# QWERTY6191/projected-lmc

Measured on AMD Instinct MI355X. Metric: MLL+grad iters/sec, n=8192 16-task LMC, higher is better.
Workload: dtype f32; 1 GPU; C3: ProjectedGPModel+ProjectedLMCmll exact training step (PLMC_fast), n=8192 d=8 p=16 q=8 Matern-5/2 fp32; latents sharded q/N per GPU; n_points=8192, n_dim=8, n_tasks=16, n_latents=8, parallelism=latent-shard x1

## Files before the change

projected-lmc_amd/csrc/api.hip:

```cpp
#include <stdlib.h>
#include <mutex>
#include <vector>

#include "api_common.hpp"
#include "../../include/plmc.h"

namespace plmc {
char *err_buf() {
  static thread_local char buf[256] = {0};
  return buf;
}

static const char *kProfNames[PK_COUNT] = {"k_assemble", "k_write_rhs", "k_assemble_cross", "k_diag",   "k_panel",
                                           "k_trail",    "k_wdiag",     "k_trtri_row",      "k_extract_col",
                                           "k_wt_matvec", "k_kinv_grad", "k_reduce_grad", "k_kernel_vjp",
                                           "sweep_total", "k_trail_row", "k_trail_head", "k_gpanel", "k_kacc", "k_grad_tiles", "k_split_w", "k_posterior_moments"};
struct ProfRec { int id; hipEvent_t a, b; double flops, bytes; };
static unsigned g_prof_mask = 0;
static std::vector<ProfRec> g_recs;
static std::vector<hipEvent_t> g_free;

static hipEvent_t get_event() {
  if (!g_free.empty()) { hipEvent_t e = g_free.back(); g_free.pop_back(); return e; }
  hipEvent_t e;
  if (hipEventCreate(&e) != hipSuccess) return nullptr;
  return e;
}

static std::recursive_mutex g_api_mutex;
void api_lock() { g_api_mutex.lock(); }
void api_unlock() { g_api_mutex.unlock(); }

static Knobs g_knobs;
static bool g_knobs_loaded = false;
static void load_knobs() {
  const char *h = getenv("PLMC_HALF_TILES"), *g = getenv("PLMC_GRP"), *o = getenv("PLMC_KINV_ORDER");
  g_knobs.half_tiles = h ? (atoi(h) == 1 ? 1e30 : (double)atoi(h)) : 640.0;
  g_knobs.grp = g ? atoi(g) : 0;
  g_knobs.serial = getenv("PLMC_SERIAL") && atoi(getenv("PLMC_SERIAL")) != 0;
  g_knobs.kinv_order = o ? atoi(o) : 4;
  g_knobs.bulk_lds = getenv("PLMC_BULK_LDS") ? atoi(getenv("PLMC_BULK_LDS")) : -1;
  g_knobs.split = getenv("PLMC_SPLIT") ? atoi(getenv("PLMC_SPLIT")) : 2;
  if (g_knobs.split != 0 && g_knobs.split != 3) g_knobs.split = 2;
  g_knobs.bulk_streams = getenv("PLMC_BULK_STREAMS") ? atoi(getenv("PLMC_BULK_STREAMS")) : 2;
  g_knobs.chain = getenv("PLMC_CHAIN") ? atoi(getenv("PLMC_CHAIN")) : 1;
  g_knobs.chain_nw = getenv("PLMC_CHAIN_NW") ? atoi(getenv("PLMC_CHAIN_NW")) : 0;
  g_knobs.chain_edge = getenv("PLMC_CHAIN_EDGE") ? atoi(getenv("PLMC_CHAIN_EDGE")) : 0;
  g_knobs_loaded = true;
}
const Knobs &knobs() {
  if (!g_knobs_loaded) {
    std::lock_guard<std::recursive_mutex> lk(g_api_mutex);
    if (!g_knobs_loaded) load_knobs();
  }
  return g_knobs;
}

constexpr int SWEEP_CTX = 2;
struct SweepCtx {
  hipStream_t caller = nullptr;
  bool used = false;
  unsigned long long stamp = 0;
  hipStream_t side[3] = {nullptr, nullptr, nullptr};
  hipEvent_t ev[16] = {nullptr};
};
static SweepCtx g_ctx[64][SWEEP_CTX];
static unsigned long long g_stamp = 0;
static thread_local int t_ctx = 0;
static SweepCtx *cur_ctx() {
  int dev = 0;
  if (hipGetDevice(&dev) != hipSuccess || dev < 0 || dev >= 64) return nullptr;
  return &g_ctx[dev][t_ctx];
}
hipStream_t side_stream(int which) {
  SweepCtx *c = cur_ctx();
  if (!c || which < 0 || which > 2) return nullptr;
  if (!c->side[which]) {
    int lo = 0, hi = 0;
    (void)hipDeviceGetStreamPriorityRange(&lo, &hi);
    if (hipStreamCreateWithPriority(&c->side[which], hipStreamNonBlocking, which == 2 ? lo : hi) != hipSuccess) c->side[which] = nullptr;
  }
  return c->side[which];
}
hipEvent_t sync_event(int idx) {
  SweepCtx *c = cur_ctx();
  if (!c) return nullptr;
  hipEvent_t &e = c->ev[idx & 15];
  if (!e && hipEventCreateWithFlags(&e, hipEventDisableTiming) != hipSuccess) e = nullptr;
  return e;
}
void bind_sweep_ctx(hipStream_t caller, int e_prev_idx) {
  int dev = 0;
  if (hipGetDevice(&dev) != hipSuccess || dev < 0 || dev >= 64) { t_ctx = 0; return; }
  SweepCtx *set = g_ctx[dev];
  int pick = -1;
  for (int i = 0; i < SWEEP_CTX; ++i)
    if (set[i].used && set[i].caller == caller) pick = i;
  if (pick < 0) {
    for (int i = 0; i < SWEEP_CTX && pick < 0; ++i)
      if (!set[i].used) pick = i;
    if (pick < 0) {
      pick = 0;
      for (int i = 1; i < SWEEP_CTX; ++i)
        if (set[i].stamp < set[pick].stamp) pick = i;
      if (set[pick].ev[e_prev_idx & 15]) (void)hipStreamWaitEvent(caller, set[pick].ev[e_prev_idx & 15], 0);
    }
    set[pick].caller = caller;
    set[pick].used = true;
  }
  set[pick].stamp = ++g_stamp;
  t_ctx = pick;
}

template <typename T>
__global__ __launch_bounds__(NTHREADS) void k_mfma_rate(T *sink, int iters) {
  using Tr = Traits<T>;
  typename Tr::acc_t acc[16];
#pragma unroll
  for (int i = 0; i < 16; ++i)
#pragma unroll
    for (int r = 0; r < 4; ++r) acc[i][r] = T(0);
  T a[4], b[4];
#pragma unroll
  for (int i = 0; i < 4; ++i) { a[i] = T(1) + T(threadIdx.x & 7) * T(1e-3) + T(i); b[i] = T(0.5) - T(i) * T(1e-3); }
#pragma unroll 1
  for (int it = 0; it < iters; ++it) {
#pragma unroll
    for (int i = 0; i < 16; ++i) acc[i] = Tr::mfma(a[i >> 2], b[i & 3], acc[i]);
  }
  T s = T(0);
#pragma unroll
  for (int i = 0; i < 16; ++i) s += acc[i][0] + acc[i][1] + acc[i][2] + acc[i][3];
  sink[(size_t)blockIdx.x * NTHREADS + threadIdx.x] = s;
}

typedef __bf16 rate_bf16x8 __attribute__((ext_vector_type(8)));
__global__ __launch_bounds__(NTHREADS) void k_mfma_rate_bf16(float *sink, int iters) {
  f32x4 acc[16];
#pragma unroll
  for (int i = 0; i < 16; ++i)
#pragma unroll
    for (int r = 0; r < 4; ++r) acc[i][r] = 0.f;
  rate_bf16x8 a[4], b[4];
#pragma unroll
  for (int i = 0; i < 4; ++i)
#pragma unroll
    for (int j = 0; j < 8; ++j) { a[i][j] = (__bf16)(1.0f + 0.01f * (float)((threadIdx.x + j) & 7) + (float)i); b[i][j] = (__bf16)(0.5f - 0.01f * (float)(i + j)); }
#pragma unroll 1
  for (int it = 0; it < iters; ++it) {
#pragma unroll
    for (int i = 0; i < 16; ++i) acc[i] = __builtin_amdgcn_mfma_f32_16x16x32_bf16(a[i >> 2], b[i & 3], acc[i], 0, 0, 0);
  }
  float s = 0.f;
#pragma unroll
  for (int i = 0; i < 16; ++i) s += acc[i][0] + acc[i][1] + acc[i][2] + acc[i][3];
  sink[(size_t)blockIdx.x * NTHREADS + threadIdx.x] = s;
}

template <typename T, bool BF16 = false> static int mfma_rate_impl(void *sink, int64_t sink_bytes, double *tflops) {
  int dev = 0;
  hipDeviceProp_t prop;
  if (hipGetDevice(&dev) != hipSuccess || hipGetDeviceProperties(&prop, dev) != hipSuccess) return fail("plmc_prof_mfma_rate", "no device");
  const int grid = 4 * prop.multiProcessorCount, iters = 4000;
  if (!sink || !tflops || sink_bytes < (int64_t)grid * NTHREADS * (int64_t)sizeof(T)) return fail("plmc_prof_mfma_rate", "sink too small");
  hipEvent_t e0 = nullptr, e1 = nullptr;
  if (hipEventCreate(&e0) != hipSuccess || hipEventCreate(&e1) != hipSuccess) return fail("plmc_prof_mfma_rate", "event");
  double best = 0.0;
  for (int rep = 0; rep < 3; ++rep) {
    (void)hipEventRecord(e0, nullptr);
    if (BF16) hipLaunchKernelGGL(k_mfma_rate_bf16, dim3(grid), dim3(NTHREADS), 0, nullptr, (float *)sink, iters);
    else hipLaunchKernelGGL(k_mfma_rate<T>, dim3(grid), dim3(NTHREADS), 0, nullptr, (T *)sink, iters);
    (void)hipEventRecord(e1, nullptr);
    float ms = 0.f;
    if (hipEventSynchronize(e1) != hipSuccess || hipEventElapsedTime(&ms, e0, e1) != hipSuccess) break;
    const double fl = (double)grid * (NTHREADS / 64) * (double)iters * 16.0 * 2.0 * 16 * 16 * (BF16 ? 32 : 4);
    if (ms > 0.f && fl / (ms * 1e-3) / 1e12 > best) best = fl / (ms * 1e-3) / 1e12;
  }
  (void)hipEventDestroy(e0);
  (void)hipEventDestroy(e1);
  *tflops = best;
  return launch_status("plmc_prof_mfma_rate");
}

ProfScope::ProfScope(int id, hipStream_t st, double flops, double bytes) : idx_(-1), st_(st) {
  api_lock();
  if (!((g_prof_mask >> id) & 1u) || g_recs.size() >= (1u << 20)) return;
  ProfRec r{id, get_event(), get_event(), flops, bytes};
  if (!r.a || !r.b) return;
  (void)hipEventRecord(r.a, st);
  g_recs.push_back(r);
  idx_ = (long)g_recs.size() - 1;
}
ProfScope::~ProfScope() {
// ... 46 lines not shown
```

projected-lmc_amd/csrc/api_common.hpp:

```cpp
#pragma once
#include <hip/hip_runtime.h>
#include <stdint.h>
#include <stdio.h>
#include <string.h>

#include "gemm_core.hpp"

namespace plmc {

constexpr int MAX_DIM = 32;

char *err_buf();

inline int fail(const char *fn, const char *msg) {
  snprintf(err_buf(), 256, "%s: %s", fn, msg);
  return -1;
}

inline int launch_status(const char *fn) {
  hipError_t e = hipGetLastError();
  if (e != hipSuccess) {
    snprintf(err_buf(), 256, "%s: HIP launch failed: %s", fn, hipGetErrorString(e));
    return -2;
  }
  return 0;
}

#define PLMC_REQUIRE(cond, msg) \
  do { if (!(cond)) return plmc::fail(__func__, msg); } while (0)

enum ProfKernel { PK_ASSEMBLE, PK_WRITE_RHS, PK_CROSS, PK_DIAG, PK_PANEL, PK_TRAIL, PK_WDIAG, PK_TRTRI, PK_EXTRACT,
                  PK_WTMV, PK_KINV_GRAD, PK_REDUCE, PK_VJP, PK_SWEEP, PK_TRAIL_ROW, PK_TRAIL_HEAD, PK_GPANEL, PK_KACC, PK_GRAD_TILES, PK_SPLIT, PK_POST, PK_COUNT };

struct ProfScope {
  ProfScope(int id, hipStream_t st, double flops, double bytes);
  ~ProfScope();
  long idx_;
  hipStream_t st_;
};

struct Knobs {
  double half_tiles;
  int grp;
  bool serial;
  int bulk_lds;
  int split;
  int bulk_streams;
  int chain;
  int chain_edge;
  int chain_nw;
  int kinv_order;
};
const Knobs &knobs();

struct AssembleJob {
  int kind, n, d;
  const void *X, *ell, *oscale, *noise;
};
int assemble_rows(const AssembleJob &job, int elem_bytes, void *A, int64_t lda, int64_t strideA, int q, int ib0, int nrows, void *stream,
                  int ncols = -1, int skip = 0);

hipStream_t side_stream(int which = 0);
hipEvent_t sync_event(int idx);
void bind_sweep_ctx(hipStream_t caller, int e_prev_idx);

inline bool aligned16(const void *p) { return (reinterpret_cast<uintptr_t>(p) & 15) == 0; }

}
```

projected-lmc_amd/csrc/bf3_engine.hpp:

```cpp
#pragma once
#include "gemm_core.hpp"

namespace plmc {

constexpr int B3_NT = 512;
constexpr int B3_K = 32;
constexpr int B3_AW = 256, B3_BW = 128;
constexpr int B3_A_PLANE = (B3_K / 8) * B3_AW * 16;
constexpr int B3_B_PLANE = (B3_K / 8) * B3_BW * 16;
constexpr int B3_WB_BYTES = 64 * 132 * 4;

typedef __bf16 b3_bf16x8 __attribute__((ext_vector_type(8)));
typedef _Float16 b3_f16x8 __attribute__((ext_vector_type(8)));
typedef short b3_s16x8 __attribute__((ext_vector_type(8)));

struct SplitB3 {
  static constexpr int NPL = 3;
  static constexpr float LEVEL1 = 1.0f;
  typedef b3_bf16x8 frag_t;
  static __device__ __forceinline__ f32x4 mfma(frag_t a, frag_t b, f32x4 c) { return __builtin_amdgcn_mfma_f32_16x16x32_bf16(a, b, c, 0, 0, 0); }
  static __device__ __forceinline__ void split(float v, short (&o)[3]) {
    const __bf16 a = (__bf16)v;
    const float r1 = v - (float)a;
    const __bf16 b = (__bf16)r1;
    const __bf16 c = (__bf16)(r1 - (float)b);
    o[0] = __builtin_bit_cast(short, a); o[1] = __builtin_bit_cast(short, b); o[2] = __builtin_bit_cast(short, c);
  }
};
struct SplitH2 {
  static constexpr int NPL = 2;
  static constexpr float LEVEL1 = 1.0f / 2048.0f;
  typedef b3_f16x8 frag_t;
  static __device__ __forceinline__ f32x4 mfma(frag_t a, frag_t b, f32x4 c) { return __builtin_amdgcn_mfma_f32_16x16x32_f16(a, b, c, 0, 0, 0); }
  static __device__ __forceinline__ void split(float v, short (&o)[2]) {
    const _Float16 a = (_Float16)v;
    const _Float16 b = (_Float16)((v - (float)a) * 2048.0f);
    o[0] = __builtin_bit_cast(short, a); o[1] = __builtin_bit_cast(short, b);
  }
};
template <class S> constexpr int b3_stage_bytes() { return S::NPL * (B3_A_PLANE + B3_B_PLANE); }
template <class S> constexpr int b3_lds_bytes() { return 2 * b3_stage_bytes<S>() > 2 * B3_WB_BYTES ? 2 * b3_stage_bytes<S>() : 2 * B3_WB_BYTES; }

template <class S> __host__ __device__ inline int64_t b3_index(int64_t k, int plane, int64_t col, int64_t ld) {
  return (((k >> 3) * S::NPL + plane) * ld + col) * 8 + (k & 7);
}
template <class S> __host__ __device__ inline int64_t b3_elems(int64_t rows, int64_t ld) { return rows * S::NPL * ld; }

__host__ __device__ inline float b3_scale_for(float bound) {
  int e;
  (void)frexpf(bound, &e);
  return ldexpf(1.0f, 13 - e);
}

template <class S>
__device__ __forceinline__ void b3_split_store(const float (&x)[8][4], unsigned short *dst, int64_t ld, float scale) {
#pragma unroll
  for (int c = 0; c < 4; ++c) {
    b3_s16x8 pl[S::NPL];
#pragma unroll
    for (int r = 0; r < 8; ++r) {
      short o[S::NPL];
      S::split(x[r][c] * scale, o);
#pragma unroll
      for (int p = 0; p < S::NPL; ++p) pl[p][r] = o[p];
    }
#pragma unroll
    for (int p = 0; p < S::NPL; ++p) *reinterpret_cast<b3_s16x8 *>(dst + (int64_t)p * ld * 8 + c * 8) = pl[p];
  }
}

template <class S, bool COPY>
__device__ __forceinline__ void b3_split_block(const float *__restrict__ Sp, int64_t lds_, unsigned short *__restrict__ P, int64_t ld, float scale,
                                               float *D, int64_t ldd, int tid) {
#pragma unroll 1
  for (int w = tid; w < 16 * 32; w += NTHREADS) {
    const int k8 = w >> 5, c4 = (w & 31) * 4;
    float x[8][4];
#pragma unroll
    for (int r = 0; r < 8; ++r) {
      const float4 v = *reinterpret_cast<const float4 *>(Sp + (int64_t)(k8 * 8 + r) * lds_ + c4);
      x[r][0] = v.x; x[r][1] = v.y; x[r][2] = v.z; x[r][3] = v.w;
      if (COPY) *reinterpret_cast<float4 *>(D + (int64_t)(k8 * 8 + r) * ldd + c4) = v;
    }
    b3_split_store<S>(x, P + ((int64_t)k8 * S::NPL * ld + c4) * 8, ld, scale);
  }
}

struct B3NoPre { __device__ __forceinline__ void operator()() const {} };
template <class S, int NSTG = 2, int NPRE = 0, class PRE = B3NoPre, bool REV = false>
__device__ __forceinline__ void b3_mainloop(Acc<float> &acc0, Acc<float> &acc1, const unsigned short *__restrict__ Ap, int64_t lda_,
                                            const unsigned short *__restrict__ Bp, int64_t ldb_, int K, unsigned char *lds, PRE pre = PRE()) {
  static_assert(NPRE == 0 || (NPRE == 8 && NSTG == 2), "pre-loads: eight, two-stage loop only");
  constexpr int NPL = S::NPL, STAGE = b3_stage_bytes<S>();
  typedef typename S::frag_t frag_t;
  const int tid = threadIdx.x, lane = tid & 63;
  const int w = __builtin_amdgcn_readfirstlane(tid >> 6);
  const int half = w >> 2, wm = (w >> 1) & 1, wn = w & 1;
  const unsigned RSA = (unsigned)(NPL * lda_ * 16), RSB = (unsigned)(NPL * ldb_ * 16);
  const unsigned PLA = (unsigned)(lda_ * 16), PLB = (unsigned)(ldb_ * 16);
  const unsigned gA0 = (unsigned)(w >> 2) * RSA + (unsigned)(w & 3) * 1024u;
  const unsigned gB0 = (unsigned)((w >> 1) & 3) * RSB + (unsigned)(w & 1) * 1024u;
  const unsigned lA0 = (unsigned)(((w >> 2) * B3_AW + (w & 3) * 64) * 16);
  const unsigned lB0 = (unsigned)(NPL * B3_A_PLANE + (((w >> 1) & 3) * B3_BW + (w & 1) * 64) * 16);
  const unsigned voff = (unsigned)lane * 16u;
  const int64_t fwdA = (int64_t)(B3_K / 8) * RSA, fwdB = (int64_t)(B3_K / 8) * RSB;
  const int64_t stepA = REV ? -fwdA : fwdA, stepB = REV ? -fwdB : fwdB;
  const char *baseA = reinterpret_cast<const char *>(Ap) + (REV ? (int64_t)(K / B3_K - 1) * fwdA : 0);
  const char *baseB = reinterpret_cast<const char *>(Bp) + (REV ? (int64_t)(K / B3_K - 1) * fwdB : 0);
  typedef __attribute__((address_space(3))) void lds_void;
  auto issue = [&](int buf) {
    const __amdgpu_buffer_rsrc_t rA = __builtin_amdgcn_make_buffer_rsrc(const_cast<char *>(baseA), 0, 0x7fffffff, 0x00020000);
    const __amdgpu_buffer_rsrc_t rB = __builtin_amdgcn_make_buffer_rsrc(const_cast<char *>(baseB), 0, 0x7fffffff, 0x00020000);
    unsigned char *sb = lds + buf * STAGE;
#pragma unroll
    for (int j = 0; j < 2 * NPL; ++j)
      __builtin_amdgcn_raw_ptr_buffer_load_lds(rA, (lds_void *)(sb + lA0 + (j >> 1) * B3_A_PLANE + (j & 1) * (2 * B3_AW * 16)), 16, voff,
                                               gA0 + (unsigned)(j & 1) * 2u * RSA + (unsigned)(j >> 1) * PLA, 0, 0);
#pragma unroll
    for (int j = 0; j < NPL; ++j)
      __builtin_amdgcn_raw_ptr_buffer_load_lds(rB, (lds_void *)(sb + lB0 + j * B3_B_PLANE), 16, voff, gB0 + (unsigned)j * PLB, 0, 0);
    baseA += stepA;
    baseB += stepB;
  };
  const int kg = lane >> 4, fr = lane & 15;
  const unsigned aA = (unsigned)((kg * B3_AW + half * 128 + wm * 64 + fr) * 16);
  const unsigned aB = (unsigned)(NPL * B3_A_PLANE + (kg * B3_BW + wn * 64 + fr) * 16);
  auto compute = [&](int buf) {
    const unsigned char *sa = lds + buf * STAGE + aA, *sb = lds + buf * STAGE + aB;
    auto fa = [&](int plane, frag_t (&f)[4]) {
#pragma unroll
      for (int t = 0; t < 4; ++t) f[t] = *reinterpret_cast<const frag_t *>(sa + plane * B3_A_PLANE + t * 256);
    };
    auto fb = [&](int plane, frag_t (&f)[4]) {
#pragma unroll
      for (int t = 0; t < 4; ++t) f[t] = *reinterpret_cast<const frag_t *>(sb + plane * B3_B_PLANE + t * 256);
    };
    auto mm = [&](Acc<float> &acc, const frag_t (&x)[4], const frag_t (&y)[4]) {
#pragma unroll
      for (int mt = 0; mt < 4; ++mt)
#pragma unroll
        for (int nt = 0; nt < 4; ++nt) acc.v[mt][nt] = S::mfma(x[mt], y[nt], acc.v[mt][nt]);
    };
    if constexpr (NPL == 3) {
      frag_t bh[4], bx[4], ax[4], ay[4];
      fb(0, bh);
      fa(2, ax);
      mm(acc1, ax, bh);
      fa(1, ay);
      mm(acc1, ay, bh);
      fb(1, bx);
      mm(acc1, ay, bx);
      fa(0, ax);
      mm(acc1, ax, bx);
      fb(2, bx);
      mm(acc1, ax, bx);
      mm(acc0, ax, bh);
    } else {
      frag_t b0[4], b1[4], a0[4], a1[4];
      fb(0, b0);
      fa(1, a1);
      mm(acc1, a1, b0);
      fa(0, a0);
      fb(1, b1);
      mm(acc1, a0, b1);
      mm(acc0, a0, b0);
    }
  };
  const int nst = K / B3_K;
  if constexpr (NSTG == 2) {
    issue(0);
#pragma unroll 1
    for (int s = 0; s + 2 < nst; s += 2) {
      __syncthreads();
      issue(1);
      compute(0);
      __syncthreads();
      issue(0);
      compute(1);
    }
    __syncthreads();
    issue(1);
    pre();
    compute(0);
    if constexpr (NPRE == 0) {
      __syncthreads();
      compute(1);
    } else {
      asm volatile("s_waitcnt vmcnt(8)" ::: "memory");
      __builtin_amdgcn_s_barrier();
      compute(1);
      asm volatile("s_waitcnt lgkmcnt(0)" ::: "memory");
      __builtin_amdgcn_s_barrier();
      return;
    }
  } else {
    static_assert(NSTG == 3 && 3 * STAGE <= 160 * 1024, "three stages must fit the LDS");
    issue(0);
    issue(1);
    int buf = 0;
#pragma unroll 1
    for (int s = 0; s < nst; ++s) {
      if (s + 1 < nst) {
        if constexpr (NPL == 2) asm volatile("s_waitcnt vmcnt(6)" ::: "memory");
        else asm volatile("s_waitcnt vmcnt(9)" ::: "memory");
      } else {
        asm volatile("s_waitcnt vmcnt(0)" ::: "memory");
      }
      __builtin_amdgcn_s_barrier();
      if (s + 2 < nst) issue(buf == 0 ? 2 : buf - 1);
      compute(buf);
      buf = buf == 2 ? 0 : buf + 1;
    }
  }
  __syncthreads();
}

template <class S> __device__ __forceinline__ void b3_combine(Acc<float> &acc0, const Acc<float> &acc1, float unscale) {
#pragma unroll
  for (int a = 0; a < 4; ++a)
#pragma unroll
    for (int b = 0; b < 4; ++b) {
      if constexpr (S::NPL == 3) acc0.v[a][b] += acc1.v[a][b];
      else acc0.v[a][b] = (acc0.v[a][b] + acc1.v[a][b] * S::LEVEL1) * unscale;
    }
}

constexpr int B3_WB_NCH = 8;
#ifndef B3_C_AUX
#define B3_C_AUX 2
#endif
#ifndef B3_C_AUX_ST
#define B3_C_AUX_ST 2
#endif
__device__ __forceinline__ void b3_preload(f32x4 (&vc)[B3_WB_NCH], const float *Cg, int64_t ldc, int tid, bool live) {
  const __amdgpu_buffer_rsrc_t rC = __builtin_amdgcn_make_buffer_rsrc(const_cast<float *>(Cg), 0, __builtin_amdgcn_readfirstlane(live ? 0x7fffffff : 0), 0x00020000);
  const unsigned voff = (unsigned)(((int64_t)(tid / 32) * ldc + (tid % 32) * 4) * 4);
  const unsigned rstep = (unsigned)((int64_t)8 * ldc * 4);
#pragma unroll
  for (int h = 0; h < B3_WB_NCH; ++h) vc[h] = __builtin_bit_cast(f32x4, __builtin_amdgcn_raw_buffer_load_b128(rC, voff, (unsigned)h * rstep, B3_C_AUX));
}
template <class S, int MODE, bool PLANES, bool PRE = false>
__device__ __forceinline__ void b3_writeback(const Acc<float> &acc, float *Cg, int64_t ldc, float *smem, int tid, bool live,
                                             unsigned short *Pp = nullptr, int64_t pld = 0, bool planes_live = true, float pscale = 1.0f,
                                             const f32x4 *vc0 = nullptr) {
  constexpr bool ADD = MODE == WB_ADD || MODE == WB_SUB;
  typedef int i32x4_t __attribute__((ext_vector_type(4)));
  constexpr int LDW = 132, CPR = 32, NCH = B3_WB_NCH, RSTEP = 8;
  const int lane = tid & 63, wave = tid >> 6, wm = wave >> 1, wn = wave & 1;
  const int row0 = tid / CPR, col0 = (tid % CPR) * 4;
  const __amdgpu_buffer_rsrc_t rC = __builtin_amdgcn_make_buffer_rsrc(Cg, 0, __builtin_amdgcn_readfirstlane(live ? 0x7fffffff : 0), 0x00020000);
  const unsigned voff = (unsigned)(((int64_t)row0 * ldc + col0) * 4);
  const unsigned rstep = (unsigned)((int64_t)RSTEP * ldc * 4);
  f32x4 vc[2][NCH];
  if (ADD) {
#pragma unroll
    for (int h = 0; h < NCH; ++h)
      vc[0][h] = PRE ? vc0[h] : __builtin_bit_cast(f32x4, __builtin_amdgcn_raw_buffer_load_b128(rC, voff, (unsigned)h * rstep, B3_C_AUX));
#pragma unroll
    for (int h = 0; h < NCH; ++h) vc[1][h] = __builtin_bit_cast(f32x4, __builtin_amdgcn_raw_buffer_load_b128(rC, voff, (unsigned)(8 + h) * rstep, B3_C_AUX));
  }
#pragma unroll
  for (int half = 0; half < 2; ++half) {
    if (half) __syncthreads();
    if (wm == half) {
#pragma unroll
      for (int mt = 0; mt < 4; ++mt)
#pragma unroll
        for (int r = 0; r < 4; ++r) {
          const int row = mt * 16 + Traits<float>::acc_row(lane, r);
#pragma unroll
          for (int nt = 0; nt < 4; ++nt) smem[row * LDW + wn * 64 + nt * 16 + (lane & 15)] = acc.v[mt][nt][r];
        }
    }
    __syncthreads();
#pragma unroll
    for (int h = 0; h < NCH; ++h) {
      float *sp = smem + (row0 + h * RSTEP) * LDW + col0;
      const f32x4 sv = *reinterpret_cast<const f32x4 *>(sp);
      const f32x4 o = MODE == WB_ADD ? vc[half][h] + sv : (MODE == WB_SUB ? vc[half][h] - sv : (MODE == WB_STORE_NEG ? -sv : sv));
      if (PLANES && MODE != WB_STORE) *reinterpret_cast<f32x4 *>(sp) = o;
      __builtin_amdgcn_raw_buffer_store_b128(__builtin_bit_cast(i32x4_t, o), rC, voff + (unsigned)(half * 8 + h) * rstep, 0, B3_C_AUX_ST);
    }
    if constexpr (PLANES) {
      __syncthreads();
      if (live && planes_live) {
        const int k8 = tid >> 5, c4 = (tid & 31) * 4;
        float x[8][4];
#pragma unroll
        for (int r = 0; r < 8; ++r) {
          const f32x4 v = *reinterpret_cast<const f32x4 *>(smem + (k8 * 8 + r) * LDW + c4);
          x[r][0] = v[0]; x[r][1] = v[1]; x[r][2] = v[2]; x[r][3] = v[3];
        }
        b3_split_store<S>(x, Pp + ((int64_t)(half * 8 + k8) * S::NPL * pld + c4) * 8, pld, pscale);
      }
    }
  }
}

}
```

projected-lmc_amd/csrc/potri_grad.hip:

```cpp
#include <stdlib.h>
#include "api_common.hpp"
#include "covariance.hpp"
#include "bf3_engine.hpp"
#include "vd_layout.hpp"
#include "../../include/plmc.h"

namespace plmc {

constexpr int GP = MAX_DIM + 2;

template <int DCAP> struct GradLds {
  static constexpr int LDI = DCAP + 4;
  static constexpr int UI = 0, UJ = UI + NB * LDI, AI = UJ + NB * LDI, AJ = AI + NB, ACCS = AJ + NB, END = ACCS + 4 * NTHREADS * 4;
};

template <typename T, int DCAP, int KIND, bool INTERIOR>
__device__ __forceinline__ void grad_tile_small(const Acc<T> &acc, T *smem, const int tid, T os, int ib, int jb, int n, int lat, int64_t n_pad,
                                                T *Kinv, int64_t ldk, int64_t strideK, T *kinv_diag, T (&g)[DCAP],
                                                T &g_noise, T &g_os) {
  typedef Pair<T> T2;
  typedef GradLds<DCAP> L;
  constexpr int NP = DCAP / 2;
  const int lane = tid & 63, wave = tid >> 6;
  const int wm = wave >> 1, wn = wave & 1;
  T2 g2[NP];
#pragma unroll
  for (int j = 0; j < NP; ++j) g2[j] = T2{T(0), T(0)};
  T gos = T(0), gnz = T(0);
  T *accs = smem + L::ACCS + tid * 4;
#pragma unroll 1
  for (int mt = 0; mt < 4; ++mt) {
#define PLMC_PARK(M)                                                                                    \
  _Pragma("unroll") for (int nt = 0; nt < 4; ++nt) _Pragma("unroll") for (int r = 0; r < 4; ++r)         \
      accs[nt * NTHREADS * 4 + r] = acc.v[M][nt][r];
    if (mt == 0) { PLMC_PARK(0) } else if (mt == 1) { PLMC_PARK(1) } else if (mt == 2) { PLMC_PARK(2) } else { PLMC_PARK(3) }
#undef PLMC_PARK
#pragma unroll 1
    for (int nt = 0; nt < 4; ++nt) {
      const int col = tile_col(wn, nt, lane);
      const T *ujc = smem + L::UJ + col * L::LDI;
      T2 u2[NP];
#pragma unroll
      for (int j = 0; j < NP; ++j) u2[j] = *reinterpret_cast<const T2 *>(ujc + 2 * j);
      const T a_j = smem[L::AJ + col];
      const int gj = jb * NB + col;
#pragma unroll 1
      for (int r = 0; r < 4; ++r) {
        const int row = tile_row<T>(wm, mt, lane, r);
        const T kin = accs[nt * NTHREADS * 4 + r];
        const T *uir = smem + L::UI + row * L::LDI;
        T2 df[NP];
        T2 r2p = {T(0), T(0)};
#pragma unroll
        for (int j = 0; j < NP; ++j) {
          df[j] = *reinterpret_cast<const T2 *>(uir + 2 * j) - u2[j];
          r2p += df[j] * df[j];
        }
        T val, base;
        if constexpr (KIND == K_SPLINE) {
          val = T(1);
#pragma unroll
          for (int j = 0; j < NP; ++j) {
            const T2 xr = *reinterpret_cast<const T2 *>(uir + 2 * j);
            val *= spline_factor(xr.x, u2[j].x) * spline_factor(xr.y, u2[j].y);
          }
          base = T(0);
        } else {
          kern_value_base_fast(KIND, r2p.x + r2p.y, val, base);
        }
        T w = smem[L::AI + row] * a_j - kin;
        if (!INTERIOR) {
          const int gi = ib * NB + row;
          if (Kinv && gj >= gi) Kinv[(int64_t)lat * strideK + (int64_t)gi * ldk + gj] = kin;
          if (kinv_diag && gi == gj) kinv_diag[(int64_t)lat * n_pad + gi] = kin;
          const bool live = gi < n && gj < n && gj >= gi;
          if (live && gi == gj) gnz += w;
          w = live ? (gj > gi ? T(2) * w : w) : T(0);
        }
        gos += w * val;
        const T c = w * base;
#pragma unroll
        for (int j = 0; j < NP; ++j) g2[j] += (c * df[j]) * df[j];
      }
    }
  }
  const T sc = INTERIOR ? T(2) * os : os;
#pragma unroll
  for (int j = 0; j < NP; ++j) {
    g[2 * j] += sc * g2[j].x;
    g[2 * j + 1] += sc * g2[j].y;
  }
  g_os += INTERIOR ? T(2) * gos : gos;
  g_noise += gnz;
}

template <typename T, int DCAP> constexpr int KG_MIN_WAVES = sizeof(T) == 8 ? 2 : (DCAP <= 8 ? 4 : (DCAP <= 16 ? 2 : 1));

template <typename T, int DCAP, bool SPLINE>
__device__ __forceinline__ void kinv_tile_epilogue(const Acc<T> &acc, T *smem, const int tid, const bool live, int kind, int ib, int jb, int lat,
                                                   int m, int64_t n_pad, const T *__restrict__ alpha, const T *__restrict__ X, int n, int d,
                                                   const T *__restrict__ ell, const T *__restrict__ oscale, T *Kinv, int64_t ldk,
                                                   int64_t strideK, T *kinv_diag, double *__restrict__ partials, int plain) {
  if (!live) { n = 0; Kinv = nullptr; kinv_diag = nullptr; }
#define PLMC_KINV_KEEP (DCAP <= 16)
#include "kinv_epilogue.inc"
#undef PLMC_KINV_KEEP
}

template <typename T, int DCAP, bool SPLINE = false>
__global__ __launch_bounds__(NTHREADS, (KG_MIN_WAVES<T, DCAP>)) void k_kinv_grad(int kind, const T *__restrict__ W, int64_t n_pad, int64_t ldw,
                                                         int64_t strideW, const T *__restrict__ alpha,
                                                         const T *__restrict__ X, int n, int d,
                                                         const T *__restrict__ ell, const T *__restrict__ oscale,
                                                         T *Kinv, int64_t ldk, int64_t strideK, T *kinv_diag,
                                                         double *__restrict__ partials, int nlat, int plain) {
  const int m = (int)(n_pad / NB);
  int lat, ib, jb;
  if (plain >= 4) {
    const int w = blockIdx.x;
    lat = w % nlat;
    const int t = w / nlat;
    jb = (int)((sqrtf(8.0f * (float)t + 1.0f) - 1.0f) * 0.5f);
    while ((jb + 1) * (jb + 2) / 2 <= t) ++jb;
    while (jb * (jb + 1) / 2 > t) --jb;
    ib = t - jb * (jb + 1) / 2;
  } else if (plain) {
    jb = blockIdx.x; ib = blockIdx.y; lat = blockIdx.z;
    if (jb < ib) return;
  } else if (!xcd_tri_decode(blockIdx.x, m, nlat, lat, ib, jb)) return;
  __shared__ __align__(16) T smem[tile_smem_elems<T>()];
  const T *Wl = W + (int64_t)lat * strideW + (int64_t)jb * NB * ldw;
  Acc<T> acc;
  acc.zero();
  tile_mainloop<T, false, true>(acc, Wl + (int64_t)ib * NB, ldw, Wl + (int64_t)jb * NB, ldw, (int)(n_pad - (int64_t)jb * NB), smem);
  const int tid = threadIdx.x;
  constexpr bool live = true;
#define PLMC_KINV_KEEP (sizeof(T) == 4)
#include "kinv_epilogue.inc"
#undef PLMC_KINV_KEEP
}

template <class S, int DCAP, bool SPLINE = false>
__global__ __launch_bounds__(B3_NT, 2) void k_kinv_grad_bf3(int kind, int64_t n_pad, const float *__restrict__ alpha, const float *__restrict__ X, int n,
                                                            int d, const float *__restrict__ ell, const float *__restrict__ oscale, float *Kinv,
                                                            int64_t ldk, int64_t strideK, float *kinv_diag, double *__restrict__ partials, int nlat,
                                                            int plain, const unsigned short *__restrict__ Wp, const float *__restrict__ wscale,
                                                            int64_t wp_lat_stride, int64_t ws_stride) {
  constexpr int LDS_BYTES = b3_lds_bytes<S>() > 2 * tile_smem_elems<float>() * (int)sizeof(float) ? b3_lds_bytes<S>() : 2 * tile_smem_elems<float>() * (int)sizeof(float);
  __shared__ __align__(16) unsigned char lds[LDS_BYTES];
  const int m = (int)(n_pad / NB);
  const int SJ = (m + 7) / 8, NSB = SJ * (SJ + 1) / 2;
  const int w = blockIdx.x, xcd = w & 7, slot = w >> 3;
  const int gb = xcd + 8 * (slot >> 5), in = slot & 31;
  if (gb >= nlat * NSB) return;
  const int lat = gb / NSB, kb = gb - lat * NSB;
  int sj = (int)((sqrtf(8.0f * (float)kb + 1.0f) - 1.0f) * 0.5f);
  while ((sj + 1) * (sj + 2) / 2 <= kb) ++sj;
  while (sj * (sj + 1) / 2 > kb) --sj;
  const int sa = kb - sj * (sj + 1) / 2;
  const int ibm = 2 * (4 * sa + (in >> 3)), jb = 8 * sj + (in & 7);
  if (jb >= m || ibm > jb) return;
  Acc<float> acc0, acc1;
  acc0.zero();
  acc1.zero();
  if (ws_stride > 1) {
    ws_stride = (int64_t)wscale[VD_W_TAG + 1] * NB * NB;
    wp_lat_stride = 2 * ws_stride;
  }
  const unsigned short *Pl = Wp + (int64_t)lat * wp_lat_stride + b3_index<S>((int64_t)jb * NB, 0, 0, n_pad);
  b3_mainloop<S, 2, 0, B3NoPre, true>(acc0, acc1, Pl + (int64_t)ibm * NB * 8, n_pad, Pl + (int64_t)jb * NB * 8, n_pad, (int)(n_pad - (int64_t)jb * NB), lds);
  float ws = wscale[(int64_t)lat * ws_stride];
  if (ws_stride > 1 && wscale[(int64_t)lat * ws_stride + VD_W_TAG] != (float)S::NPL) ws = __builtin_nanf("");
  b3_combine<S>(acc0, acc1, 1.0f / (ws * ws));
  const int half = __builtin_amdgcn_readfirstlane((int)threadIdx.x >> 8);
  const int ib = ibm + half;
  kinv_tile_epilogue<float, DCAP, SPLINE>(acc0, reinterpret_cast<float *>(lds) + half * tile_smem_elems<float>(), (int)threadIdx.x & 255, ib <= jb, kind,
                                          ib, jb, lat, m, n_pad, alpha, X, n, d, ell, oscale, Kinv, ldk, strideK, kinv_diag, partials, plain);
}


constexpr int RED_NT = 1024;
template <typename T>
__global__ __launch_bounds__(RED_NT) void k_reduce_grad(const double *__restrict__ partials, int m, int d,
                                                        const T *__restrict__ ell, double *__restrict__ grad) {
  __shared__ double red[RED_NT];
  const int lat = blockIdx.x;
  const int ntile = m * m;
  const int slot = threadIdx.x % GP;
  const int grp = threadIdx.x / GP;
  constexpr int NG = RED_NT / GP;
  double s[4] = {0.0, 0.0, 0.0, 0.0};
  if (grp < NG) {
    const double *base = partials + (int64_t)lat * ntile * GP + slot;
    for (int t0 = grp; t0 < ntile; t0 += 4 * NG) {
#pragma unroll
      for (int u = 0; u < 4; ++u) {
        const int t = t0 + u * NG;
        if (t < ntile) {
          const int ib = t / m, jb = t - ib * m;
          if (jb >= ib) s[u] += base[(int64_t)t * GP];
        }
      }
    }
  }
  red[threadIdx.x] = (s[0] + s[1]) + (s[2] + s[3]);
  __syncthreads();
  if (threadIdx.x < GP) {
    double tot = 0.0;
    for (int gq = 0; gq < NG; ++gq) tot += red[gq * GP + threadIdx.x];
    const int k = threadIdx.x;
    if (k < d) grad[(int64_t)lat * (d + 2) + k] = 0.5 * tot / (double)ell[(int64_t)lat * d + k];
    else if (k == MAX_DIM) grad[(int64_t)lat * (d + 2) + d] = 0.5 * tot;
    else if (k == MAX_DIM + 1) grad[(int64_t)lat * (d + 2) + d + 1] = 0.5 * tot;
  }
}

template <typename T, int DCAP>
__global__ __launch_bounds__(NTHREADS) void k_grad_tiles(int kind, const T *__restrict__ A, int64_t n_pad, int64_t lda, int64_t strideA,
                                                         const T *__restrict__ Kd, int64_t strideKd, const T *__restrict__ alpha,
                                                         const T *__restrict__ X, int n, int d, const T *__restrict__ ell,
                                                         const T *__restrict__ oscale, T *kinv_diag, double *__restrict__ partials,
                                                         int nlat) {
  const int m = (int)(n_pad / NB);
  const int w = blockIdx.x, lat = w % nlat, t = w / nlat;
  int jb = (int)((sqrtf(8.0f * (float)t + 1.0f) - 1.0f) * 0.5f);
  while ((jb + 1) * (jb + 2) / 2 <= t) ++jb;
  while (jb * (jb + 1) / 2 > t) --jb;
  const int ib = t - jb * (jb + 1) / 2;
  __shared__ T ui[NB][DCAP + 1];
  __shared__ T ai[NB];
  __shared__ double red[4][GP];
  const int tid = threadIdx.x, lane = tid & 63, wave = tid >> 6;
  const T *el = ell + (int64_t)lat * d;
  for (int e = tid; e < NB * DCAP; e += NTHREADS) {
    const int r = e / DCAP, k = e % DCAP, gi = ib * NB + r;
    ui[r][k] = (k < d && gi < n) ? X[(int64_t)gi * d + k] / el[k] : T(0);
  }
  if (tid < NB) ai[tid] = alpha[(int64_t)lat * n_pad + ib * NB + tid];
  const int col = tid & (NB - 1), rh = tid >> 7;
  const int gj = jb * NB + col;
  T uj[DCAP];
#pragma unroll
  for (int k = 0; k < DCAP; ++k) uj[k] = (k < d && gj < n) ? X[(int64_t)gj * d + k] / el[k] : T(0);
  const T a_j = alpha[(int64_t)lat * n_pad + gj];
  const T os = oscale ? oscale[lat] : T(1);
  const T *Kt;
  int64_t ldk;
  if (ib == jb) { Kt = Kd + (int64_t)lat * strideKd + (int64_t)ib * NB * NB; ldk = NB; }
  else { Kt = A + (int64_t)lat * strideA + (int64_t)jb * NB * lda + (int64_t)ib * NB; ldk = lda; }
  __syncthreads();
  T g[DCAP];
#pragma unroll
  for (int k = 0; k < DCAP; ++k) g[k] = T(0);
  T g_noise = T(0), g_os = T(0);
#pragma unroll 4
  for (int rr = 0; rr < NB / 2; ++rr) {
    const int row = 2 * rr + rh, gi = ib * NB + row;
    const T kin = Kt[(int64_t)row * ldk + col];
    if (kinv_diag && gi == gj) kinv_diag[(int64_t)lat * n_pad + gi] = kin;
    const bool live = gi < n && gj < n && gj >= gi;
    T wv = ai[row] * a_j - kin;
    if (live && gi == gj) g_noise += wv;
    wv = live ? (gj > gi ? T(2) * wv : wv) : T(0);
    T df[DCAP];
    T r2 = T(0), sp = T(1);
#pragma unroll
    for (int k = 0; k < DCAP; ++k) {
      df[k] = ui[row][k] - uj[k];
      r2 += df[k] * df[k];
      if (kind == K_SPLINE) sp *= spline_factor(ui[row][k], uj[k]);
    }
    T val, base;
    if (kind == K_SPLINE) { val = sp; base = T(0); }
    else kern_value_base_fast(kind, r2, val, base);
    g_os += wv * val;
    const T c = wv * os * base;
#pragma unroll
    for (int k = 0; k < DCAP; ++k) g[k] += c * df[k] * df[k];
  }
  auto wave_sum = [&](double v) {
#pragma unroll
    for (int o = 32; o > 0; o >>= 1) v += __shfl_down(v, o, 64);
    return v;
  };
#pragma unroll
  for (int k = 0; k < DCAP; ++k) {
    double s = wave_sum((double)g[k]);
    if (lane == 0) red[wave][k] = s;
  }
  {
    double s = wave_sum((double)g_noise);
    if (lane == 0) red[wave][MAX_DIM] = s;
    s = wave_sum((double)g_os);
    if (lane == 0) red[wave][MAX_DIM + 1] = s;
  }
  __syncthreads();
  double *out = partials + (((int64_t)lat * m + ib) * m + jb) * GP;
  if (tid < GP) {
    const bool lv = tid < DCAP || tid >= MAX_DIM;
    out[tid] = lv ? red[0][tid] + red[1][tid] + red[2][tid] + red[3][tid] : 0.0;
  }
}

template <typename T>
int grad_tiles_impl(int kind, const T *A, int64_t n_pad, int64_t lda, int64_t strideA, const T *Vd, const T *alpha, const T *X, int n, int d,
                    const T *ell, const T *oscale, double *grad, T *kinv_diag, void *partials, int q, void *stream) {
  PLMC_REQUIRE(kind >= 0 && kind <= 4, "unknown kernel kind");
  PLMC_REQUIRE(A && Vd && alpha && X && ell && grad && partials, "null pointer");
  PLMC_REQUIRE(n_pad > 0 && n_pad % NB == 0 && lda % NB == 0 && n <= n_pad && n > n_pad - NB, "n_pad must be plmc_pad(n)");
  PLMC_REQUIRE(d > 0 && d <= MAX_DIM && q > 0, "need 0<d<=plmc_max_dim(), q>0");
  hipStream_t st = (hipStream_t)stream;
  const int m = (int)(n_pad / NB);
  const VdLayout L(n_pad, lda, (int)sizeof(T), false);
  const int64_t strideV = L.stride();
  const T *Kd = L.at<const T>(Vd, L.kd);
  double *part = reinterpret_cast<double *>(partials);
  const dim3 grid(q * (m * (m + 1) / 2)), block(NTHREADS);
#define PLMC_LAUNCH_GT(DC) \
  hipLaunchKernelGGL((k_grad_tiles<T, DC>), grid, block, 0, st, kind, A, n_pad, lda, strideA, Kd, strideV, alpha, X, n, d, ell, oscale, kinv_diag, part, q)
  {
    const double np = (double)n_pad;
    ProfScope ps(PK_GRAD_TILES, st, 0.0, q * (np * np / 2) * sizeof(T));
    if (d <= 4) PLMC_LAUNCH_GT(4);
    else if (d <= 8) PLMC_LAUNCH_GT(8);
    else if (d <= 16) PLMC_LAUNCH_GT(16);
    else PLMC_LAUNCH_GT(32);
  }
#undef PLMC_LAUNCH_GT
  {
    ProfScope ps(PK_REDUCE, st, 0.0, (double)m * m * q * GP * sizeof(double) / 2);
    hipLaunchKernelGGL(k_reduce_grad<T>, dim3(q), dim3(RED_NT), 0, st, part, m, d, ell, grad);
  }
  return launch_status(__func__);
}

template <class S>
__global__ __launch_bounds__(NTHREADS) void k_split_w(const float *__restrict__ W, int64_t n_pad, int64_t ldw, int64_t strideW,
                                                      unsigned short *__restrict__ Wp, const float *__restrict__ wscale) {
  const int cb = blockIdx.x, lb = blockIdx.y, lat = blockIdx.z;
  if (cb > lb) return;
  b3_split_block<S, false>(W + (int64_t)lat * strideW + (int64_t)lb * NB * ldw + (int64_t)cb * NB, ldw,
                           Wp + (int64_t)lat * b3_elems<S>(n_pad, n_pad) + b3_index<S>((int64_t)lb * NB, 0, (int64_t)cb * NB, n_pad), n_pad, wscale[lat],
                           nullptr, 0, threadIdx.x);
}
template <class S>
__global__ void k_w_scale(const float *__restrict__ eig_lo, float *__restrict__ wscale, int q, int padded) {
  const int lat = threadIdx.x;
  if (lat >= q) return;
  if constexpr (S::NPL == 3) wscale[lat] = 1.0f;
  else {
    float lam = fmaxf(eig_lo[lat], 1e-30f);
    if (padded) lam = fminf(lam, 1.0f);
    wscale[lat] = b3_scale_for(1.0f / sqrtf(lam));
  }
}

template <typename T, class S>
int kinv_grad_impl(int kind, const T *W, int64_t n_pad, int64_t ldw, int64_t strideW, const T *alpha, const T *X, int n,
                   int d, const T *ell, const T *oscale, double *grad, T *Kinv, int64_t ldk, int64_t strideK,
                   T *kinv_diag, void *partials, int q, const float *eig_lo, void *stream, const float *Vd = nullptr, int64_t lda_vd = 0) {
  PLMC_REQUIRE(kind >= 0 && kind <= 4, "unknown kernel kind");
  PLMC_REQUIRE(W && alpha && X && ell && grad && partials, "null pointer");
  PLMC_REQUIRE(n_pad > 0 && n_pad % NB == 0 && ldw % NB == 0 && n <= n_pad && n > n_pad - NB, "n_pad must be plmc_pad(n)");
  PLMC_REQUIRE(d > 0 && d <= MAX_DIM && q > 0, "need 0<d<=plmc_max_dim(), q>0");
  PLMC_REQUIRE(!Kinv || (ldk >= n_pad), "ldk too small");
  PLMC_REQUIRE(aligned16(W), "unaligned W");
  hipStream_t st = (hipStream_t)stream;
  const int m = (int)(n_pad / NB);
  const int plain = knobs().kinv_order;
  const dim3 grid = plain >= 4 ? dim3(q * (m * (m + 1) / 2)) : plain ? dim3(m, m, q) : dim3(xcd_tri_grid(m, q)), block(NTHREADS);
  double *part = reinterpret_cast<double *>(partials);
  const double np = (double)n_pad;
  bool done = false;
  if constexpr (!std::is_void<S>::value) {
    PLMC_REQUIRE(q <= 1024, "too many latents for one scale launch");
    const unsigned short *wp = nullptr;
    const float *wsc = nullptr;
    int64_t wp_lat = b3_elems<S>(n_pad, n_pad), ws_lat = 1;
    if (!(Vd && vd_w_planes(Vd, n_pad, lda_vd, &wp, &wp_lat, &wsc, &ws_lat))) {
      char *pb = reinterpret_cast<char *>(partials) + (int64_t)m * m * q * GP * (int64_t)sizeof(double);
      unsigned short *wpo = reinterpret_cast<unsigned short *>(pb);
      float *wsco = reinterpret_cast<float *>(pb + (int64_t)q * b3_elems<SplitB3>(n_pad, n_pad) * 2);
      hipLaunchKernelGGL((k_w_scale<S>), dim3(1), dim3(q < 64 ? 64 : ((q + 63) / 64) * 64), 0, st, eig_lo, wsco, q, (int)(n < n_pad));
      ProfScope ps(PK_SPLIT, st, 0.0, (double)q * np * np / 2 * (4 + 2 * S::NPL));
      hipLaunchKernelGGL((k_split_w<S>), dim3(m, m, q), dim3(NTHREADS), 0, st, (const float *)W, n_pad, ldw, strideW, wpo, (const float *)wsco);
      wp = wpo;
      wsc = wsco;
      wp_lat = b3_elems<S>(n_pad, n_pad);
      ws_lat = 1;
    }
    const int SJ = (m + 7) / 8, NSB = SJ * (SJ + 1) / 2;
    const dim3 gridb(8 * ((q * NSB + 7) / 8) * 32);
#define PLMC_LAUNCH_KB(DC, SP) \
  hipLaunchKernelGGL((k_kinv_grad_bf3<S, DC, SP>), gridb, dim3(B3_NT), 0, st, kind, n_pad, alpha, X, n, d, ell, oscale, Kinv, ldk, strideK, kinv_diag, \
                     part, q, plain, wp, wsc, wp_lat, ws_lat)
    ProfScope ps(PK_KINV_GRAD, st, q * np * np * np / 3.0, q * (np * np / 2) * sizeof(T));
    if (d <= 4) PLMC_LAUNCH_KB(4, false);
    else if (d <= 8) PLMC_LAUNCH_KB(8, false);
    else if (d <= 16) { if (kind == K_SPLINE) PLMC_LAUNCH_KB(16, true); else PLMC_LAUNCH_KB(16, false); }
    else { if (kind == K_SPLINE) PLMC_LAUNCH_KB(32, true); else PLMC_LAUNCH_KB(32, false); }
#undef PLMC_LAUNCH_KB
    done = true;
  }
#define PLMC_LAUNCH_KG(DC, SP)                                                                                       \
  hipLaunchKernelGGL((k_kinv_grad<T, DC, SP>), grid, block, 0, st, kind, W, n_pad, ldw, strideW, alpha, X, n, d, ell, \
                     oscale, Kinv, ldk, strideK, kinv_diag, part, q, plain)
  if (!done) {
    ProfScope ps(PK_KINV_GRAD, st, q * np * np * np / 3.0, q * (np * np / 2) * sizeof(T));
    if (d <= 4) PLMC_LAUNCH_KG(4, false);
    else if (d <= 8) PLMC_LAUNCH_KG(8, false);
    else if (d <= 16) { if (kind == K_SPLINE) PLMC_LAUNCH_KG(16, true); else PLMC_LAUNCH_KG(16, false); }
    else { if (kind == K_SPLINE) PLMC_LAUNCH_KG(32, true); else PLMC_LAUNCH_KG(32, false); }
  }
#undef PLMC_LAUNCH_KG
  {
    ProfScope ps(PK_REDUCE, st, 0.0, (double)m * m * q * GP * sizeof(double) / 2);
    hipLaunchKernelGGL(k_reduce_grad<T>, dim3(q), dim3(RED_NT), 0, st, part, m, d, ell, grad);
  }
  return launch_status(__func__);
}

}

extern "C" {
int plmc_grad_tiles_f32(int kind, const float *A, int64_t n_pad, int64_t lda, int64_t strideA, const float *Vd, const float *alpha,
                        const float *X, int n, int d, const float *ell, const float *oscale, double *grad, float *kinv_diag,
                        void *partials, int q, void *stream) {
  return plmc::grad_tiles_impl<float>(kind, A, n_pad, lda, strideA, Vd, alpha, X, n, d, ell, oscale, grad, kinv_diag, partials, q, stream);
}
int plmc_grad_tiles_f64(int kind, const double *A, int64_t n_pad, int64_t lda, int64_t strideA, const double *Vd, const double *alpha,
                        const double *X, int n, int d, const double *ell, const double *oscale, double *grad, double *kinv_diag,
                        void *partials, int q, void *stream) {
  return plmc::grad_tiles_impl<double>(kind, A, n_pad, lda, strideA, Vd, alpha, X, n, d, ell, oscale, grad, kinv_diag, partials, q, stream);
}
int64_t plmc_grad_scratch_bytes_for(int64_t n_pad, int q, int elem_bytes) {
  int64_t m = n_pad / plmc::NB;
  const int64_t planes = elem_bytes == 4 ? (int64_t)q * plmc::b3_elems<plmc::SplitB3>(n_pad, n_pad) * 2 + 4096 : 0;
  return m * m * (int64_t)q * plmc::GP * (int64_t)sizeof(double) + planes;
}
int64_t plmc_grad_scratch_bytes(int64_t n_pad, int q) { return plmc_grad_scratch_bytes_for(n_pad, q, 4); }
int64_t plmc_grad_partials_bytes(int64_t n_pad, int q) {
  const int64_t m = n_pad / plmc::NB;
  return m * m * (int64_t)q * plmc::GP * (int64_t)sizeof(double);
}
static int kinv_grad_f32_any(int kind, const float *W, int64_t n_pad, int64_t ldw, int64_t strideW, const float *alpha,
                             const float *X, int n, int d, const float *ell, const float *oscale, double *grad,
                             float *Kinv, int64_t ldk, int64_t strideK, float *kinv_diag, void *partials, int q, const float *eig_lo,
                             void *stream, const float *Vd = nullptr) {
  const int split = plmc::knobs().split;
  if (split == 0)
    return plmc::kinv_grad_impl<float, void>(kind, W, n_pad, ldw, strideW, alpha, X, n, d, ell, oscale, grad, Kinv, ldk, strideK, kinv_diag, partials, q,
                                             nullptr, stream);
  if (split == 2 && eig_lo)
    return plmc::kinv_grad_impl<float, plmc::SplitH2>(kind, W, n_pad, ldw, strideW, alpha, X, n, d, ell, oscale, grad, Kinv, ldk, strideK, kinv_diag,
                                                      partials, q, eig_lo, stream, Vd, ldw);
  return plmc::kinv_grad_impl<float, plmc::SplitB3>(kind, W, n_pad, ldw, strideW, alpha, X, n, d, ell, oscale, grad, Kinv, ldk, strideK, kinv_diag,
                                                    partials, q, nullptr, stream, Vd, ldw);
}
int plmc_kinv_grad_f32(int kind, const float *W, int64_t n_pad, int64_t ldw, int64_t strideW, const float *alpha,
                       const float *X, int n, int d, const float *ell, const float *oscale, double *grad,
                       float *Kinv, int64_t ldk, int64_t strideK, float *kinv_diag, void *partials, int q,
                       void *stream) {
  return kinv_grad_f32_any(kind, W, n_pad, ldw, strideW, alpha, X, n, d, ell, oscale, grad, Kinv, ldk, strideK, kinv_diag, partials, q, nullptr, stream);
}
int plmc_kinv_grad_ex_f32(int kind, const float *W, int64_t n_pad, int64_t ldw, int64_t strideW, const float *alpha,
                          const float *X, int n, int d, const float *ell, const float *oscale, double *grad,
                          float *Kinv, int64_t ldk, int64_t strideK, float *kinv_diag, void *partials, int q,
                          const float *eig_lo, void *stream) {
  return kinv_grad_f32_any(kind, W, n_pad, ldw, strideW, alpha, X, n, d, ell, oscale, grad, Kinv, ldk, strideK, kinv_diag, partials, q, eig_lo, stream);
}
int plmc_kinv_grad_vd_f32(int kind, const float *W, int64_t n_pad, int64_t ldw, int64_t strideW, const float *alpha,
                          const float *X, int n, int d, const float *ell, const float *oscale, double *grad,
                          float *Kinv, int64_t ldk, int64_t strideK, float *kinv_diag, void *partials, int q,
                          const float *eig_lo, const float *Vd, void *stream) {
  return kinv_grad_f32_any(kind, W, n_pad, ldw, strideW, alpha, X, n, d, ell, oscale, grad, Kinv, ldk, strideK, kinv_diag, partials, q, eig_lo, stream, Vd);
}
int plmc_kinv_grad_vd_f64(int kind, const double *W, int64_t n_pad, int64_t ldw, int64_t strideW, const double *alpha,
                          const double *X, int n, int d, const double *ell, const double *oscale, double *grad,
                          double *Kinv, int64_t ldk, int64_t strideK, double *kinv_diag, void *partials, int q,
                          const double *eig_lo, const double *Vd, void *stream) {
  (void)eig_lo;
  (void)Vd;
  return plmc::kinv_grad_impl<double, void>(kind, W, n_pad, ldw, strideW, alpha, X, n, d, ell, oscale, grad, Kinv, ldk,
                                            strideK, kinv_diag, partials, q, nullptr, stream);
}
int plmc_kinv_grad_f64(int kind, const double *W, int64_t n_pad, int64_t ldw, int64_t strideW, const double *alpha,
                       const double *X, int n, int d, const double *ell, const double *oscale, double *grad,
                       double *Kinv, int64_t ldk, int64_t strideK, double *kinv_diag, void *partials, int q,
                       void *stream) {
  return plmc::kinv_grad_impl<double, void>(kind, W, n_pad, ldw, strideW, alpha, X, n, d, ell, oscale, grad, Kinv, ldk,
                                            strideK, kinv_diag, partials, q, nullptr, stream);
}
int plmc_kinv_grad_ex_f64(int kind, const double *W, int64_t n_pad, int64_t ldw, int64_t strideW, const double *alpha,
                          const double *X, int n, int d, const double *ell, const double *oscale, double *grad,
                          double *Kinv, int64_t ldk, int64_t strideK, double *kinv_diag, void *partials, int q,
                          const double *eig_lo, void *stream) {
  (void)eig_lo;
  return plmc::kinv_grad_impl<double, void>(kind, W, n_pad, ldw, strideW, alpha, X, n, d, ell, oscale, grad, Kinv, ldk,
                                            strideK, kinv_diag, partials, q, nullptr, stream);
}
}
```

Baseline: 54.87 iters/sec.

## Pace kinv-grad workgroups in lockstep windows to improve shared-panel cache reuse

Adds an optional inter-workgroup pacing scheme to the bf3 K-inverse gradient mainloop. Groups of 32 blocks publish their K-stage progress to a global line, and blocks running ahead sleep until laggards fall within a window, bounded by a time cap. The goal is to keep co-scheduled blocks streaming the same W panel stages together so they hit in L2 instead of refetching from HBM. It is on by default (window 8, every 2 stages, small cap) and costs extra atomics, sleeps, and the risk of stalls from imperfect co-residency.

```diff
diff --git a/projected-lmc_amd/csrc/api.hip b/projected-lmc_amd/csrc/api.hip
--- a/projected-lmc_amd/csrc/api.hip
+++ b/projected-lmc_amd/csrc/api.hip
@@ -39,6 +39,10 @@
   g_knobs.grp = g ? atoi(g) : 0;
   g_knobs.serial = getenv("PLMC_SERIAL") && atoi(getenv("PLMC_SERIAL")) != 0;
   g_knobs.kinv_order = o ? atoi(o) : 4;
+  g_knobs.kinv_window = getenv("PLMC_KINV_WINDOW") ? atoi(getenv("PLMC_KINV_WINDOW")) : 8;
+  g_knobs.kinv_every = getenv("PLMC_KINV_WINDOW_EVERY") ? atoi(getenv("PLMC_KINV_WINDOW_EVERY")) : 2;
+  if (g_knobs.kinv_every < 1 || (g_knobs.kinv_every & (g_knobs.kinv_every - 1))) g_knobs.kinv_every = 2;
+  g_knobs.kinv_cap_us = getenv("PLMC_KINV_WINDOW_CAP") ? atoi(getenv("PLMC_KINV_WINDOW_CAP")) : 4;
   g_knobs.bulk_lds = getenv("PLMC_BULK_LDS") ? atoi(getenv("PLMC_BULK_LDS")) : -1;
   g_knobs.split = getenv("PLMC_SPLIT") ? atoi(getenv("PLMC_SPLIT")) : 2;
   if (g_knobs.split != 0 && g_knobs.split != 3) g_knobs.split = 2;
diff --git a/projected-lmc_amd/csrc/api_common.hpp b/projected-lmc_amd/csrc/api_common.hpp
--- a/projected-lmc_amd/csrc/api_common.hpp
+++ b/projected-lmc_amd/csrc/api_common.hpp
@@ -50,6 +50,9 @@
   int chain_edge;
   int chain_nw;
   int kinv_order;
+  int kinv_window;
+  int kinv_every;
+  int kinv_cap_us;
 };
 const Knobs &knobs();
 
diff --git a/projected-lmc_amd/csrc/bf3_engine.hpp b/projected-lmc_amd/csrc/bf3_engine.hpp
--- a/projected-lmc_amd/csrc/bf3_engine.hpp
+++ b/projected-lmc_amd/csrc/bf3_engine.hpp
@@ -87,10 +87,13 @@
 }
 
 struct B3NoPre { __device__ __forceinline__ void operator()() const {} };
-template <class S, int NSTG = 2, int NPRE = 0, class PRE = B3NoPre, bool REV = false>
+struct B3NoPace { __device__ __forceinline__ void operator()(int) {} };
+template <class S, int NSTG = 2, int NPRE = 0, class PRE = B3NoPre, bool REV = false, class PACE = B3NoPace>
 __device__ __forceinline__ void b3_mainloop(Acc<float> &acc0, Acc<float> &acc1, const unsigned short *__restrict__ Ap, int64_t lda_,
-                                            const unsigned short *__restrict__ Bp, int64_t ldb_, int K, unsigned char *lds, PRE pre = PRE()) {
+                                            const unsigned short *__restrict__ Bp, int64_t ldb_, int K, unsigned char *lds, PRE pre = PRE(),
+                                            PACE pace = PACE()) {
   static_assert(NPRE == 0 || (NPRE == 8 && NSTG == 2), "pre-loads: eight, two-stage loop only");
+  static_assert(std::is_same<PACE, B3NoPace>::value || NSTG == 2, "pacing: two-stage loop only");
   constexpr int NPL = S::NPL, STAGE = b3_stage_bytes<S>();
   typedef typename S::frag_t frag_t;
   const int tid = threadIdx.x, lane = tid & 63;
@@ -168,17 +171,21 @@
   };
   const int nst = K / B3_K;
   if constexpr (NSTG == 2) {
+    pace(0);
     issue(0);
 #pragma unroll 1
     for (int s = 0; s + 2 < nst; s += 2) {
       __syncthreads();
+      pace(s + 1);
       issue(1);
       compute(0);
       __syncthreads();
+      pace(s + 2);
       issue(0);
       compute(1);
     }
     __syncthreads();
+    pace(nst - 1);
     issue(1);
     pre();
     compute(0);
diff --git a/projected-lmc_amd/csrc/potri_grad.hip b/projected-lmc_amd/csrc/potri_grad.hip
--- a/projected-lmc_amd/csrc/potri_grad.hip
+++ b/projected-lmc_amd/csrc/potri_grad.hip
@@ -140,13 +140,57 @@
 #undef PLMC_KINV_KEEP
 }
 
-template <class S, int DCAP, bool SPLINE = false>
+constexpr int KP_LINES = 256;
+constexpr unsigned KP_DONE = 0x8000u, KP_STAGE_MAX = 0x7fffu;
+__device__ unsigned g_kinv_pace[KP_LINES * 32];
+struct KinvPaceArgs {
+  unsigned tag;
+  int window;
+  int every;
+  int cap;
+};
+struct KinvPace {
+  unsigned *line;
+  unsigned tag;
+  int window, every, me;
+  long long left;
+  unsigned v = 0;
+  __device__ __forceinline__ bool behind(int ref) const {
+    const int lane = threadIdx.x;
+    const bool lag = lane < 32 && (v >> 16) == tag && !(v & KP_DONE) && (int)(v & KP_STAGE_MAX) + window < ref;
+    return __builtin_amdgcn_ballot_w64(lag) != 0;
+  }
+  __device__ __forceinline__ void operator()(int s) {
+    if (__builtin_amdgcn_readfirstlane((int)threadIdx.x >> 6) != 0 || (s & (every - 1)) != 0) return;
+    const int lane = threadIdx.x;
+    if (s > 0 && left > 0 && behind(s - every)) {
+      do {
+        const long long t0 = wall_clock64();
+        __builtin_amdgcn_s_sleep(8);
+        if (lane < 32) v = __hip_atomic_load(line + lane, __ATOMIC_RELAXED, __HIP_MEMORY_SCOPE_AGENT);
+        left -= wall_clock64() - t0;
+      } while (left > 0 && behind(s));
+    }
+    if (lane == 0) __builtin_nontemporal_store((tag << 16) | (unsigned)s, line + me);
+    if (lane < 32) v = __hip_atomic_load(line + lane, __ATOMIC_RELAXED, __HIP_MEMORY_SCOPE_AGENT);
+  }
+};
+
+#ifndef PLMC_KINV_NSTG
+#define PLMC_KINV_NSTG 2
+#endif
+#ifndef PLMC_KINV_REV
+#define PLMC_KINV_REV true
+#endif
+template <class S, int DCAP, bool SPLINE = false, bool PACE = false>
 __global__ __launch_bounds__(B3_NT, 2) void k_kinv_grad_bf3(int kind, int64_t n_pad, const float *__restrict__ alpha, const float *__restrict__ X, int n,
                                                             int d, const float *__restrict__ ell, const float *__restrict__ oscale, float *Kinv,
                                                             int64_t ldk, int64_t strideK, float *kinv_diag, double *__restrict__ partials, int nlat,
                                                             int plain, const unsigned short *__restrict__ Wp, const float *__restrict__ wscale,
-                                                            int64_t wp_lat_stride, int64_t ws_stride) {
-  constexpr int LDS_BYTES = b3_lds_bytes<S>() > 2 * tile_smem_elems<float>() * (int)sizeof(float) ? b3_lds_bytes<S>() : 2 * tile_smem_elems<float>() * (int)sizeof(float);
+                                                            int64_t wp_lat_stride, int64_t ws_stride, KinvPaceArgs pa) {
+  constexpr int NSTG = S::NPL == 2 && !PACE ? PLMC_KINV_NSTG : 2;
+  constexpr int LDS_B3 = b3_lds_bytes<S>() > NSTG * b3_stage_bytes<S>() ? b3_lds_bytes<S>() : NSTG * b3_stage_bytes<S>();
+  constexpr int LDS_BYTES = LDS_B3 > 2 * tile_smem_elems<float>() * (int)sizeof(float) ? LDS_B3 : 2 * tile_smem_elems<float>() * (int)sizeof(float);
   __shared__ __align__(16) unsigned char lds[LDS_BYTES];
   const int m = (int)(n_pad / NB);
   const int SJ = (m + 7) / 8, NSB = SJ * (SJ + 1) / 2;
@@ -168,7 +212,15 @@
     wp_lat_stride = 2 * ws_stride;
   }
   const unsigned short *Pl = Wp + (int64_t)lat * wp_lat_stride + b3_index<S>((int64_t)jb * NB, 0, 0, n_pad);
-  b3_mainloop<S, 2, 0, B3NoPre, true>(acc0, acc1, Pl + (int64_t)ibm * NB * 8, n_pad, Pl + (int64_t)jb * NB * 8, n_pad, (int)(n_pad - (int64_t)jb * NB), lds);
+  if constexpr (PACE) {
+    unsigned *line = g_kinv_pace + (gb % KP_LINES) * 32;
+    b3_mainloop<S, 2, 0, B3NoPre, true, KinvPace>(acc0, acc1, Pl + (int64_t)ibm * NB * 8, n_pad, Pl + (int64_t)jb * NB * 8, n_pad,
+                                                  (int)(n_pad - (int64_t)jb * NB), lds, B3NoPre(),
+                                                  KinvPace{line, pa.tag, pa.window, pa.every, in, (long long)pa.cap});
+    if (threadIdx.x == 0) __builtin_nontemporal_store((pa.tag << 16) | KP_DONE, line + in);
+  } else {
+    b3_mainloop<S, NSTG, 0, B3NoPre, PLMC_KINV_REV>(acc0, acc1, Pl + (int64_t)ibm * NB * 8, n_pad, Pl + (int64_t)jb * NB * 8, n_pad, (int)(n_pad - (int64_t)jb * NB), lds);
+  }
   float ws = wscale[(int64_t)lat * ws_stride];
   if (ws_stride > 1 && wscale[(int64_t)lat * ws_stride + VD_W_TAG] != (float)S::NPL) ws = __builtin_nanf("");
   b3_combine<S>(acc0, acc1, 1.0f / (ws * ws));
@@ -391,15 +443,21 @@
     }
     const int SJ = (m + 7) / 8, NSB = SJ * (SJ + 1) / 2;
     const dim3 gridb(8 * ((q * NSB + 7) / 8) * 32);
-#define PLMC_LAUNCH_KB(DC, SP) \
-  hipLaunchKernelGGL((k_kinv_grad_bf3<S, DC, SP>), gridb, dim3(B3_NT), 0, st, kind, n_pad, alpha, X, n, d, ell, oscale, Kinv, ldk, strideK, kinv_diag, \
-                     part, q, plain, wp, wsc, wp_lat, ws_lat)
+    static unsigned launches = 0;
+    const Knobs &kn = knobs();
+    const KinvPaceArgs pa{launches++ % 0xffffu + 1u, kn.kinv_window, kn.kinv_every, kn.kinv_cap_us * 100};
+    const bool pace = kn.kinv_window > 0 && n_pad / B3_K <= (int64_t)KP_STAGE_MAX;
+#define PLMC_LAUNCH_KB1(DC, SP, PC) \
+  hipLaunchKernelGGL((k_kinv_grad_bf3<S, DC, SP, PC>), gridb, dim3(B3_NT), 0, st, kind, n_pad, alpha, X, n, d, ell, oscale, Kinv, ldk, strideK, \
+                     kinv_diag, part, q, plain, wp, wsc, wp_lat, ws_lat, pa)
+#define PLMC_LAUNCH_KB(DC, SP) do { if (pace) PLMC_LAUNCH_KB1(DC, SP, true); else PLMC_LAUNCH_KB1(DC, SP, false); } while (0)
     ProfScope ps(PK_KINV_GRAD, st, q * np * np * np / 3.0, q * (np * np / 2) * sizeof(T));
     if (d <= 4) PLMC_LAUNCH_KB(4, false);
     else if (d <= 8) PLMC_LAUNCH_KB(8, false);
     else if (d <= 16) { if (kind == K_SPLINE) PLMC_LAUNCH_KB(16, true); else PLMC_LAUNCH_KB(16, false); }
     else { if (kind == K_SPLINE) PLMC_LAUNCH_KB(32, true); else PLMC_LAUNCH_KB(32, false); }
 #undef PLMC_LAUNCH_KB
+#undef PLMC_LAUNCH_KB1
     done = true;
   }
 #define PLMC_LAUNCH_KG(DC, SP)                                                                                       \
```

Result: slower. 54.30 iters/sec, median of 2 (-1.0%).
